# colmap/pycolmap

Measured on AMD Instinct MI355X. Metric: descriptor-pair distances/sec (exhaustive SIFT match: dot + top-2 + ratio + cross-check), higher is better.
Workload: dtype u8 descriptors, int8 MFMA / int32 accumulate; 1 GPU; 500 images x 4096 descriptors, exhaustive match + ratio test + cross-check (BASELINE.json configs[1] at N=1); pairs_total=124750, pairs_per_rank=124750, kernel=auto, matches_rank0=1865611

## Files before the change

### pycolmap_amd/csrc/match_mfma.hip

```cpp
#include <cstdlib>

#include "amc_internal.h"
#include "scan_accept.h"

namespace amc {

typedef int i32x4 __attribute__((ext_vector_type(4)));
typedef __attribute__((address_space(1))) const void gvoid_t;
typedef __attribute__((address_space(3))) void lvoid_t;

constexpr int kBN = 256;
constexpr int kYS = kBN / 32;
constexpr int kUR = 128;
constexpr int kSPB = kUR / 32;
constexpr int kUPC = kBN / kUR;
constexpr int kChunkBytes = kBN * kDim;
constexpr int kW = kSegsPerItem;
constexpr int kXT = kSegRows / 16;
constexpr int kKeyShift = 7, kKeyCarried = 127;

constexpr int kNB = 3;
constexpr int kOffRs = 0;
constexpr int kOffQ = kOffRs + kNB * kBN * 4;
constexpr int kOffB = kOffQ + 16;
constexpr int kLdsBytes = kOffB + kNB * kChunkBytes;
static_assert(kBN == kRowPad, "a chunk is the row padding unit");
static_assert(kUR == 128 && kSPB == 4, "a lane quarter's rows of a block are one 32-row tile; the loop body is one block");
static_assert(kRowPad % kSegRows == 0 && kSegRows % 32 == 0, "segments tile the padded rows");
static_assert(kLdsBytes <= 160 * 1024, "LDS of one CU");
static_assert(sizeof(SegDesc) == 64, "a descriptor is 16 dwords: one per lane of a quarter wave");

enum : int { kDXprep = 0, kDXrs = 2, kDOut = 4, kDList = 6, kDYprep = 8, kDYrs = 10, kDCnt = 12, kDAccword = 13,
             kDYrows = 14 };

__device__ __forceinline__ void mfma_first(i32x4& d, const i32x4& a, const i32x4& b, const i32x4& c) {
    asm volatile("v_mfma_i32_16x16x64_i8 %0, %1, %2, %3" : "=&v"(d) : "v"(a), "v"(b), "v"(c));
}
__device__ __forceinline__ void mfma_acc(i32x4& d, const i32x4& a, const i32x4& b) {
    asm volatile("v_mfma_i32_16x16x64_i8 %0, %1, %2, %0" : "+v"(d) : "v"(a), "v"(b));
}

struct YFrag {
    i32x4 f[2][2];
    i32x4 ci[2];
};

#ifdef AMC_SCAN_STAMPS
constexpr int kStampMaxWG = 1024;
__device__ uint32_t g_scan_stamps[2 * kStampMaxWG * kSegsPerItem * 8];
#define AMC_STAMP() ((uint32_t)__builtin_amdgcn_s_memtime())
#endif

__device__ __noinline__ __attribute__((used)) void copy_part(const uint4* __restrict__ src, uint4* __restrict__ dst,
                                                             unsigned long long b, unsigned long long e, int tid,
                                                             int nthreads) {
    __builtin_assume(tid >= 0 && tid < 1024 && nthreads >= 256 && nthreads <= 512);
    unsigned long long i = b + (unsigned long long)tid;
    const unsigned long long st = (unsigned long long)nthreads;
    for (; i + 3 * st < e; i += 4 * st) {
        const uint4 v0 = src[i], v1 = src[i + st], v2 = src[i + 2 * st], v3 = src[i + 3 * st];
        dst[i] = v0; dst[i + st] = v1; dst[i + 2 * st] = v2; dst[i + 3 * st] = v3;
    }
    for (; i < e; i += st) dst[i] = src[i];
}

template <int MODE>
__global__ __launch_bounds__(64 * kW) void match_mfma_kernel(const SegDesc* __restrict__ segs,
                                                             const uint32_t* __restrict__ nitems_p,
                                                             uint32_t* __restrict__ queue_head,
                                                             uint32_t* __restrict__ accmask,
                                                             const ScanAccept* __restrict__ accept,
                                                             CopyJob job, uint32_t* __restrict__ copy_head) {
    static_assert((kChunkBytes / 1024) % kW == 0 && kYS % (kChunkBytes / 1024 / kW) == 0, "a chunk splits into 1 KiB DMA pieces per wave, dealt evenly over its steps");
    __shared__ __attribute__((aligned(16))) char smem[kLdsBytes];

    const int tid = threadIdx.x;
    const int lane = tid & 63;
    const int wid = __builtin_amdgcn_readfirstlane(tid >> 6);
    const int l15 = lane & 15, lq = lane >> 4;
    volatile uint32_t* s_q = reinterpret_cast<volatile uint32_t*>(smem + kOffQ);
    if constexpr (MODE == 0) {
        if (job.parts) {
            __shared__ uint32_t s_part;
            if (tid == 0) s_part = atomicAdd(copy_head, 1u);
            __syncthreads();
            const uint32_t part = s_part;
            if (part < job.parts)
                copy_part(static_cast<const uint4*>(job.src), static_cast<uint4*>(job.dst), job.n16 * part / job.parts,
                          job.n16 * (part + 1) / job.parts, tid, 64 * kW);
        }
    }
    const uint32_t nitems = *nitems_p;
    const ScanAccept sa = *accept;

    auto load_desc = [&](uint32_t q) -> int {
        int v = 0;
        if (q < nitems && lane < 16) v = reinterpret_cast<const int*>(segs + (size_t)q * kSegsPerItem + wid)[lane];
        return v;
    };
    auto dword = [&](int dv, int f) -> int { return __builtin_amdgcn_readlane(dv, f); };
    auto dptr = [&](int dv, int f) -> const char* {
        const uint64_t lo = (uint32_t)__builtin_amdgcn_readlane(dv, f);
        const uint64_t hi = (uint32_t)__builtin_amdgcn_readlane(dv, f + 1);
        return reinterpret_cast<const char*>(lo | (hi << 32));
    };

    constexpr int kPW = kChunkBytes / 1024 / kW;
    auto stage_piece = [&](const char* yprep, int c, int buf, int ps) __attribute__((always_inline)) {
        const int piece = ps * kW + wid;
        __builtin_amdgcn_global_load_lds((gvoid_t*)(yprep + (size_t)c * kChunkBytes + piece * 1024 + lane * 16),
                                         (lvoid_t*)(smem + kOffB + buf * kChunkBytes + piece * 1024), 16, 0, 0);
    };
    auto stage_rs = [&](const char* yrs, int c, int buf) __attribute__((always_inline)) {
        if (wid == 0)
            __builtin_amdgcn_global_load_lds((gvoid_t*)(yrs + (size_t)c * kBN * 4 + lane * 16),
                                             (lvoid_t*)(smem + kOffRs + buf * kBN * 4), 16, 0, 0);
    };
    auto stage = [&](const char* yprep, const char* yrs, int c, int buf) __attribute__((always_inline)) {
#pragma unroll
        for (int ps = 0; ps < kPW; ++ps) stage_piece(yprep, c, buf, ps);
        stage_rs(yrs, c, buf);
    };

    const int yrow_lane = (kUR / 4) * (l15 >> 2) + (l15 & 3);
    const int ysw_lane = arena_swizzle(yrow_lane);
    const int yoff0 = kOffB + yrow_lane * kDim + ((lq ^ ysw_lane) * 16);
    const int yoff1 = kOffB + yrow_lane * kDim + (((4 + lq) ^ ysw_lane) * 16);
    const int coff = kOffRs + (kUR / 4) * lq * 4;
    auto load_y_part = [&](YFrag& y, int buf, int ys, int part) __attribute__((always_inline)) {
        const int ub = (ys / kSPB) * kUR, sp = ys % kSPB;
        if (part < 2) {
            const int so = buf * kBN * 4 + (ub + 8 * sp) * 4;
            y.ci[part] = *reinterpret_cast<const i32x4*>(smem + (coff + so) + 16 * part);
        } else {
            const int tt = (part - 2) >> 1, s = (part - 2) & 1;
            const int so = buf * kChunkBytes + (ub + 8 * sp) * kDim;
            y.f[tt][s] = *reinterpret_cast<const i32x4*>(smem + ((s ? yoff1 : yoff0) + so) + tt * 4 * kDim);
        }
    };
    auto load_y = [&](YFrag& y, int buf, int ys) __attribute__((always_inline)) {
#pragma unroll
        for (int part = 0; part < 6; ++part) load_y_part(y, buf, ys, part);
    };

    i32x4 xf[kXT][2];
    int best[kXT], sec[kXT], btile[kXT], xterm[kXT], part[kXT];
    auto load_x = [&](int dv) __attribute__((always_inline)) {
        const int cnt = dword(dv, kDCnt);
        const char* xprep = dptr(dv, kDXprep);
        const int* xrs = reinterpret_cast<const int*>(dptr(dv, kDXrs));
#pragma unroll
        for (int xt = 0; xt < kXT; ++xt) {
            const int kl = xt * 16 + l15;
            int row;
            if (MODE == 0) {
                row = kl;
            } else {
                const uint32_t* list = reinterpret_cast<const uint32_t*>(dptr(dv, kDList));
                row = cnt > 0 ? (int)list[min(kl, cnt - 1)] : 0;
            }
            const char* rp = xprep + (size_t)row * kDim;
            const int sw = arena_swizzle(row);
#pragma unroll
            for (int s = 0; s < 2; ++s) xf[xt][s] = *reinterpret_cast<const i32x4*>(rp + (((4 * s + lq) ^ sw) * 16));
            xterm[xt] = xrs[row] - (1 << 21);
            best[xt] = ((-xterm[xt]) << kKeyShift) | kKeyCarried;
            sec[xt] = best[xt];
            btile[xt] = -1;
        }
    };

#ifdef AMC_SCAN_STAMPS
    uint32_t st_a = 0, st_first = 0, st_end = 0, st_sum[5] = {0, 0, 0, 0, 0};
    bool st_prev = false, st_prev_active = false;
    uint32_t* const st_slot = g_scan_stamps + ((size_t)(MODE * kStampMaxWG + min((int)blockIdx.x, kStampMaxWG - 1)) * kW + wid) * 8;
#endif
    if (tid == 0) *s_q = atomicAdd(queue_head, 1u);
    __syncthreads();
    uint32_t q = *s_q;
    int dv = load_desc(q);
    if (q < nitems) {
        stage(dptr(dv, kDYprep), dptr(dv, kDYrs), 0, 0);
        if (dword(dv, kDYrows) > kBN) stage(dptr(dv, kDYprep), dptr(dv, kDYrs), 1, 1);
        if (dword(dv, kDCnt) > 0) load_x(dv);
    }
    __syncthreads();

    while (q < nitems) {
        const char* yprep = dptr(dv, kDYprep);
        const char* yrs = dptr(dv, kDYrs);
        const int yrows_item = dword(dv, kDYrows);
        const int nchunks = (yrows_item + kBN - 1) / kBN;
        const int last_steps = (((yrows_item - (nchunks - 1) * kBN) + 31) / 32 + kSPB - 1) & ~(kSPB - 1);
        const bool active = dword(dv, kDCnt) > 0;
        if (tid == 0) *s_q = atomicAdd(queue_head, 1u);

        i32x4 acc[2][2];
        auto insert = [&](int xt, int code) __attribute__((always_inline)) {
            asm volatile(
                "v_lshl_or_b32 %2, %2, 7, %3\n\t"
                "v_med3_i32 %1, %0, %1, %2\n\t"
                "v_max_i32 %0, %0, %2"
                : "+v"(best[xt]), "+v"(sec[xt]), "+v"(part[xt])
                : "s"(code));
        };
        auto flush = [&](int sb) __attribute__((always_inline)) {
#pragma unroll
            for (int xt = 0; xt < kXT; ++xt) {
                const int c = best[xt] & 127;
                btile[xt] = c != kKeyCarried ? sb * 64 + (126 - c) : btile[xt];
                best[xt] |= kKeyCarried;
            }
        };
        auto phase = [&](i32x4 (&an)[2], const YFrag& y, int xtn, const i32x4 (&ac)[2], int xtc, int sp, int gb)
                         __attribute__((always_inline)) {
            mfma_first(an[0], y.f[0][0], xf[xtn][0], y.ci[0]);
            mfma_first(an[1], y.f[1][0], xf[xtn][0], y.ci[1]);
            __builtin_amdgcn_sched_barrier(0);
            if (xtc == 0 ? sp == 0 : sp == kSPB - 1) {
                insert((xtc + kXT - 1) % kXT, 126 - ((xtc == 0 ? gb - 1 : gb) & 63));
                if (xtc == 0 && gb != 0 && (gb & 63) == 0) flush((gb >> 6) - 1);
                __builtin_amdgcn_sched_barrier(0);
            }
            mfma_acc(an[0], y.f[0][1], xf[xtn][1]);
            mfma_acc(an[1], y.f[1][1], xf[xtn][1]);
            __builtin_amdgcn_sched_barrier(0);
            int t0, t1;
            if (sp == 0)
                asm volatile(
                    "v_max3_i32 %0, %3, %4, %5\n\t"
                    "v_max3_i32 %1, %6, %7, %8\n\t"
                    "v_max3_i32 %0, %0, %9, %10\n\t"
                    "v_max_i32 %2, %0, %1"
                    : "=&v"(t0), "=&v"(t1), "=&v"(part[xtc])
                    : "v"(ac[0][0]), "v"(ac[0][1]), "v"(ac[0][2]), "v"(ac[0][3]), "v"(ac[1][0]), "v"(ac[1][1]),
                      "v"(ac[1][2]), "v"(ac[1][3]));
            else
                asm volatile(
                    "v_max3_i32 %0, %3, %4, %5\n\t"
                    "v_max3_i32 %1, %6, %7, %8\n\t"
                    "v_max3_i32 %0, %0, %9, %10\n\t"
                    "v_max3_i32 %2, %0, %1, %2"
                    : "=&v"(t0), "=&v"(t1), "+v"(part[xtc])
                    : "v"(ac[0][0]), "v"(ac[0][1]), "v"(ac[0][2]), "v"(ac[0][3]), "v"(ac[1][0]), "v"(ac[1][1]),
                      "v"(ac[1][2]), "v"(ac[1][3]));
            __builtin_amdgcn_sched_barrier(0);
        };

        YFrag y0, y1;
        asm volatile("s_waitcnt vmcnt(0)" ::: "memory");
        __syncthreads();
        const uint32_t qn = *s_q;
        const int dvn = load_desc(qn);
#ifdef AMC_SCAN_STAMPS
        {
            const uint32_t now = AMC_STAMP();
            if (st_prev) {
                st_sum[0] += st_a;
                st_sum[1] += now - st_end;
                st_sum[2] += now - st_first;
                st_sum[3] += 1;
                st_sum[4] += st_prev_active ? 1 : 0;
                if (lane == 0) {
#pragma unroll
                    for (int k = 0; k < 5; ++k) st_slot[k] = st_sum[k];
                }
            }
            st_a = 0;
            st_first = now;
        }
#endif
        if (active) {
            load_y(y0, 0, 0);
            mfma_first(acc[0][0], y0.f[0][0], xf[0][0], y0.ci[0]);
            mfma_first(acc[0][1], y0.f[1][0], xf[0][0], y0.ci[1]);
            mfma_acc(acc[0][0], y0.f[0][1], xf[0][1]);
            mfma_acc(acc[0][1], y0.f[1][1], xf[0][1]);
            part[kXT - 1] = -(1 << 24);
            __builtin_amdgcn_sched_barrier(0);
        }
        auto step = [&](YFrag& yc, YFrag& yn, int c, int cb, int nb, int ys, int sp) __attribute__((always_inline)) {
            const bool lastt = sp == kSPB - 1 && ys == kYS - 1;
            const bool cross = lastt && (c + 1 < nchunks);
            const bool fetch = c + 2 < nchunks;
            if (fetch) {
                const int fb = cb == 0 ? 2 : cb - 1;
                constexpr int kEvery = kYS / kPW;
                static_assert(kEvery == 2, "a DMA piece behind every other step");
                if (sp % kEvery == 0) stage_piece(yprep, c + 2, fb, ys / kEvery);
                if (ys == 0) stage_rs(yrs, c + 2, fb);
            }
            if (cross) {
#ifdef AMC_SCAN_STAMPS
                const uint32_t st_t = AMC_STAMP();
#endif
                if (!fetch) asm volatile("s_waitcnt vmcnt(0)" ::: "memory");
                else if (wid == 0) asm volatile("s_waitcnt vmcnt(%0)" ::"n"(kPW + 1) : "memory");
                else asm volatile("s_waitcnt vmcnt(%0)" ::"n"(kPW) : "memory");
                asm volatile("s_barrier" ::: "memory");
#ifdef AMC_SCAN_STAMPS
                st_a += AMC_STAMP() - st_t;
#endif
            }
            if (active) {
                const int nbuf = cross ? nb : cb;
                const int nys = lastt ? (cross ? 0 : ys) : ys + 1;
                const int gb = c * kUPC + ys / kSPB;
#pragma unroll
                for (int xt = 0; xt < kXT; ++xt) {
                    if (xt + 1 < kXT)
                        phase(acc[(xt + 1) & 1], yc, xt + 1, acc[xt & 1], xt, sp, gb);
                    else
                        phase(acc[0], yn, 0, acc[xt & 1], xt, sp, gb);
                    if (xt < 6) {
                        load_y_part(yn, nbuf, nys, xt);
                        __builtin_amdgcn_sched_barrier(0);
                    }
                }
            }
        };
        for (int c = 0, cb = 0; c < nchunks; ++c) {
            const int nb = cb == 2 ? 0 : cb + 1;
            const int yend = (c == nchunks - 1) ? last_steps : kYS;
#pragma unroll 1
            for (int ys = 0; ys < yend; ys += kSPB) {
                step(y0, y1, c, cb, nb, ys, 0);
                step(y1, y0, c, cb, nb, ys + 1, 1);
                step(y0, y1, c, cb, nb, ys + 2, 2);
                step(y1, y0, c, cb, nb, ys + 3, 3);
            }
            cb = nb;
        }
        if (active) {
            const int lastb = (nchunks - 1) * kUPC + last_steps / kSPB - 1;
            insert(kXT - 1, 126 - (lastb & 63));
            flush(lastb >> 6);
#pragma unroll
            for (int xt = 0; xt < kXT; ++xt) {
                best[xt] >>= kKeyShift;
                sec[xt] >>= kKeyShift;
            }
        }
        __syncthreads();
#ifdef AMC_SCAN_STAMPS
        st_end = AMC_STAMP();
        st_prev = true;
        st_prev_active = active;
#endif

        int eb[kXT], es[kXT], et[kXT], ex[kXT];
#pragma unroll
        for (int xt = 0; xt < kXT; ++xt) {
            asm volatile("v_mov_b32 %0, %1" : "=v"(eb[xt]) : "v"(best[xt]));
            asm volatile("v_mov_b32 %0, %1" : "=v"(es[xt]) : "v"(sec[xt]));
            asm volatile("v_mov_b32 %0, %1" : "=v"(et[xt]) : "v"(btile[xt]));
            ex[xt] = xterm[xt];
        }
        if (qn < nitems) {
            stage(dptr(dvn, kDYprep), dptr(dvn, kDYrs), 0, 0);
            if (dword(dvn, kDYrows) > kBN) stage(dptr(dvn, kDYprep), dptr(dvn, kDYrs), 1, 1);
            if (dword(dvn, kDCnt) > 0) load_x(dvn);
        }
        if (active) {
            const int cnt = dword(dv, kDCnt);
            uint32_t bits_lo = 0;
#pragma unroll
            for (int xt = 0; xt < kXT; ++xt) {
                const int kl = xt * 16 + l15;
                int b = eb[xt], s = es[xt], t = et[xt] < 0 ? -1 : et[xt] * kSPB + lq;
#pragma unroll
                for (int m = 16; m <= 32; m <<= 1) {
                    const int ob = __shfl_xor(b, m);
                    const int os = __shfl_xor(s, m);
                    const int ot = __shfl_xor(t, m);
                    const bool ow = (ob > b) || (ob == b && (unsigned)ot < (unsigned)t);
                    s = max(max(s, os), ow ? b : ob);
                    t = ow ? ot : t;
                    b = ow ? ob : b;
                }
                bool acc_bit = false;
                const bool live = lq == 0 && kl < cnt;
                Top2 o;
                o.best_v = (uint32_t)(b + ex[xt]);
                o.best_idx = o.best_v ? (uint32_t)t : 0xFFFFFFFFu;
                o.second_v = (uint32_t)(s + ex[xt]);
                o.pad = 0;
                if (MODE == 0) acc_bit = live && scan_may_accept(sa, o.best_v, o.second_v);
                const uint32_t bits = MODE == 0 ? (uint32_t)__ballot(acc_bit) : 0u;
                if (live && (MODE == 1 || bits != 0)) {
                    Top2* out = reinterpret_cast<Top2*>(const_cast<char*>(dptr(dv, kDOut)));
                    int row = kl;
                    if (MODE == 1) row = (int)reinterpret_cast<const uint32_t*>(dptr(dv, kDList))[kl];
                    out[row] = o;
                }
                if (MODE == 0) {
                    if (xt & 1) {
                        const uint32_t word = bits_lo | (bits << 16);
                        if (lane == 0 && word != 0) accmask[(uint32_t)dword(dv, kDAccword) + (xt >> 1)] = word;
                    } else {
                        bits_lo = bits;
                    }
                }
            }
        }
#ifdef AMC_SCAN_STAMPS
        if (qn >= nitems && lane == 0) {
            st_slot[5] = st_a;
            st_slot[6] = AMC_STAMP() - st_first;
            st_slot[7] = 1;
        }
#endif
        q = qn;
        dv = dvn;
    }
}

__device__ __forceinline__ uint32_t pair_segments(int mode, const ImageDev* imgs, const PairDev& p, uint32_t pi,
                                                  const uint32_t* cand_cnt, uint32_t* nrows_out) {
    const uint32_t nx = mode == 0 ? imgs[p.slot1].rows : cand_cnt[pi];
    const uint32_t ny = imgs[mode == 0 ? p.slot2 : p.slot1].rows;
    *nrows_out = nx;
    return ny ? (nx + kSegRows - 1) / kSegRows : 0u;
}

__global__ __launch_bounds__(256) void seg_count_kernel(int mode, const ImageDev* __restrict__ imgs,
                                                        const PairDev* __restrict__ pairs,
                                                        const uint32_t* __restrict__ order,
                                                        const uint32_t* __restrict__ grp_start,
                                                        const uint32_t* __restrict__ cand_cnt,
                                                        uint32_t* __restrict__ seg_base, uint32_t* __restrict__ grp_segs) {
    __shared__ uint32_t wsum[4];
    const uint32_t g = blockIdx.x, tid = threadIdx.x, lane = tid & 63, wid = tid >> 6;
    const uint32_t i0 = grp_start[g], i1 = grp_start[g + 1];
    uint32_t running = 0;
    for (uint32_t base = i0; base < i1; base += 256) {
        const uint32_t i = base + tid;
        uint32_t s = 0, nr;
        if (i < i1) {
            const uint32_t pi = order[i];
            s = pair_segments(mode, imgs, pairs[pi], pi, cand_cnt, &nr);
        }
        uint32_t inc = s;
#pragma unroll
// ... 54 lines not shown
                                                       const uint32_t* __restrict__ seg_base,
                                                       const uint32_t* __restrict__ grp_segs,
                                                       const uint32_t* __restrict__ grp_item_base,
                                                       Top2* __restrict__ outbuf, SegDesc* __restrict__ segs) {
    const uint32_t g = blockIdx.x, tid = threadIdx.x, lane = tid & 63, wid = blockIdx.y * 4 + (tid >> 6);
    const uint32_t i0 = grp_start[g], i1 = grp_start[g + 1];
    if (i0 >= i1) return;
    const uint32_t total = grp_segs[g];
    if (total == 0) return;
    SegDesc* gs = segs + (size_t)grp_item_base[g] * kSegsPerItem;
    const PairDev p0 = pairs[order[i0]];
    const ImageDev Y = imgs[mode == 0 ? p0.slot2 : p0.slot1];
    for (uint32_t i = i0 + wid; i < i1; i += 4 * kFillY) {
        const uint32_t pi = order[i];
        const PairDev p = pairs[pi];
        uint32_t nx;
        const uint32_t ns = pair_segments(mode, imgs, p, pi, cand_cnt, &nx);
        const ImageDev X = imgs[mode == 0 ? p.slot1 : p.slot2];
        const uint32_t sb = seg_base[i];
        for (uint32_t k = lane; k < ns; k += 64) {
            const uint32_t row0 = k * kSegRows;
            SegDesc d;
            d.yprep = Y.prep;
            d.yrs = Y.rs128;
            d.yrows = Y.rows;
            d.cnt = min(nx - row0, (uint32_t)kSegRows);
            d.pad_ = 0;
            if (mode == 0) {
                d.xprep = X.prep + (size_t)row0 * kDim;
                d.xrs = X.rs128 + row0;
                d.out = outbuf + p.row_off + row0;
                d.list = nullptr;
                d.accword = (uint32_t)((p.row_off + row0) >> 5);
            } else {
                d.xprep = X.prep;
                d.xrs = X.rs128;
                d.out = outbuf + p.col_off;
                d.list = candbuf + p.col_off + row0;
                d.accword = 0;
            }
            gs[sb + k] = d;
        }
    }
    const uint32_t padded = (total + kSegsPerItem - 1) / kSegsPerItem * kSegsPerItem;
    if (blockIdx.y == 0 && tid < padded - total) {
        SegDesc d;
        d.xprep = Y.prep;
        d.xrs = Y.rs128;
        d.out = nullptr;
        d.list = nullptr;
        d.yprep = Y.prep;
        d.yrs = Y.rs128;
        d.cnt = 0;
        d.accword = 0;
        d.yrows = Y.rows;
        d.pad_ = 0;
        gs[total + tid] = d;
    }
}

hipError_t launch_build_segments(int mode, const ImageDev* imgs, const PairDev* pairs, const uint32_t* order,
                                 const uint32_t* grp_start, uint32_t ngroups, const uint32_t* cand_cnt,
                                 const uint32_t* candbuf, Top2* outbuf, uint32_t* seg_base, uint32_t* grp_segs,
                                 uint32_t* grp_item_base, SegDesc* segs, uint32_t* nitems_dev, hipStream_t s) {
    if (ngroups == 0) return memset_async(nitems_dev, 0, sizeof(uint32_t), s);
    hipLaunchKernelGGL(seg_count_kernel, dim3(ngroups), dim3(256), 0, s, mode, imgs, pairs, order, grp_start,
                       cand_cnt, seg_base, grp_segs);
    hipLaunchKernelGGL(seg_scan_kernel, dim3(1), dim3(1024), 0, s, grp_segs, ngroups, grp_item_base, nitems_dev);
    hipLaunchKernelGGL(seg_fill_kernel, dim3(ngroups, kFillY), dim3(256), 0, s, mode, imgs, pairs, order, grp_start,
                       cand_cnt, candbuf, seg_base, grp_segs, grp_item_base, outbuf, segs);
    return hipGetLastError();
}

hipError_t launch_match_mfma(int mode, const SegDesc* segs, const uint32_t* nitems_dev, uint32_t max_items,
                             uint32_t* queue_head, uint32_t* accmask, const ScanAccept* accept_dev, hipStream_t s,
                             const CopyJob& job_in, uint32_t* copy_head) {
    if (max_items == 0) return hipSuccess;
    CopyJob job = (mode == 0 && copy_head) ? job_in : CopyJob();
    hipError_t e = job.parts ? memset_async(copy_head, 0, sizeof(uint32_t), s) : hipSuccess;
    if (e != hipSuccess) return e;
    int dev = 0, cus = 256;
    if ((e = hipGetDevice(&dev)) != hipSuccess) return e;
    if ((e = hipDeviceGetAttribute(&cus, hipDeviceAttributeMultiprocessorCount, dev)) != hipSuccess) return e;
    static const int grid_cap = [] {
        const char* e = std::getenv("AMC_SCAN_GRID");
        return e ? std::atoi(e) : 0;
    }();
    if (grid_cap > 0 && grid_cap < cus) cus = grid_cap;
    const uint32_t grid = max_items < (uint32_t)cus ? max_items : (uint32_t)cus;
    if (job.parts > grid) job.parts = grid;
    if ((e = memset_async(queue_head, 0, sizeof(uint32_t), s)) != hipSuccess) return e;
    if (mode == 0)
        hipLaunchKernelGGL((match_mfma_kernel<0>), dim3(grid), dim3(64 * kW), 0, s, segs, nitems_dev, queue_head,
                           accmask, accept_dev, job, copy_head);
    else
        hipLaunchKernelGGL((match_mfma_kernel<1>), dim3(grid), dim3(64 * kW), 0, s, segs, nitems_dev, queue_head,
                           accmask, accept_dev, job, copy_head);
    return hipGetLastError();
}

}
```

### pycolmap_amd/csrc/amc_internal.h

```cpp
#pragma once

#include <hip/hip_runtime.h>
#include <stdint.h>

#include <algorithm>
#include <cstdlib>
#include <type_traits>
#include <vector>

#include "../../include/amc.h"
#include "guided_region.h"

namespace amc {

constexpr int kDim = AMC_DESC_DIM;
constexpr int kRowPad = 256;
constexpr int kAcosLutSize = 262145;

__host__ __device__ __forceinline__ constexpr uint32_t arena_swizzle(uint32_t row) {
    return ((row >> 1) & 1u) | (((row >> 5) & 3u) << 1);
}

struct ImageDev {
    const uint8_t* raw;
// ... 196 lines not shown

    hipError_t start() { return made_ != hipSuccess ? made_ : hipEventRecord(ab_[0], s_); }
    hipError_t stop(double& ms) {
        hipError_t e = hipEventRecord(ab_[1], s_);
        if (e == hipSuccess) e = hipEventSynchronize(ab_[1]);
        return e == hipSuccess ? add_elapsed(ab_[0], ab_[1], ms) : e;
    }
    hipError_t span_begin() {
        hipEvent_t two[2];
        if (const hipError_t e = create_events(two, 2)) return e;
        spans_.insert(spans_.end(), two, two + 2);
        return hipEventRecord(two[0], s_);
    }
    hipError_t span_end() { return hipEventRecord(spans_.back(), s_); }
    hipError_t spans(double& ms) const {
        for (size_t i = 0; i + 1 < spans_.size(); i += 2)
            if (const hipError_t e = add_elapsed(spans_[i], spans_[i + 1], ms)) return e;
        return hipSuccess;
    }

  private:
    static hipError_t add_elapsed(hipEvent_t a, hipEvent_t b, double& ms) {
        float f = 0.f;
        const hipError_t e = hipEventElapsedTime(&f, a, b);
        if (e == hipSuccess) ms += f;
        return e;
    }
    hipStream_t s_;
    hipEvent_t ab_[2] = {nullptr, nullptr};
    hipError_t made_;
    std::vector<hipEvent_t> spans_;
};

struct Batches {
    std::vector<size_t> start{0};
    uint64_t most_items = 0, most_elems = 0;
    size_t count() const { return start.size() - 1; }
};
inline Batches split_batches(const uint64_t* offsets, size_t n, uint64_t max_items, uint64_t max_elems,
                             uint64_t factor = 1) {
    Batches b;
    for (size_t i = 0; i < n;) {
        size_t j = i + 1;
        while (j < n && j - i < max_items && (offsets[j + 1] - offsets[i]) * factor <= max_elems) ++j;
        b.most_items = std::max<uint64_t>(b.most_items, j - i);
        b.most_elems = std::max<uint64_t>(b.most_elems, offsets[j] - offsets[i]);
        b.start.push_back(j);
        i = j;
    }
    return b;
}

struct CtxView {
    int device;
    hipStream_t stream;
    const uint32_t* resident;
    uint64_t resident_rows;
};
CtxView ctx_view(amc_ctx* c);
struct TvgPair;
struct VerifyResident {
    size_t npairs = 0;
    uint64_t total = 0;
    const amc_tvg* tvg = nullptr;
    const uint8_t* mask = nullptr;
    const uint64_t* moff = nullptr;
    const TvgPair* tp = nullptr;
    const uint32_t* matches = nullptr;
};
VerifyResident verify_resident(amc_ctx* c);

hipError_t memset_async(void* p, int value, size_t bytes, hipStream_t s);
hipError_t memcpy_async(void* dst, const void* src, size_t bytes, hipMemcpyKind kind, hipStream_t s);

hipError_t launch_prep(const uint8_t* raw, uint8_t* prep, int32_t* rs128, uint32_t rows_pad,
                 uint32_t* maxsq_out, hipStream_t s);

hipError_t launch_match_dot4(const ImageDev* imgs, const PairDev* pairs, const Dot4Work* work,
                       uint32_t nwork, Top2* rowbuf, Top2* colbuf, const GuidedDev* guided, hipStream_t s);
hipError_t launch_match_guided_grid(const ImageDev* imgs, const GridDev* grids, const PairDev* pairs, const Dot4Work* work,
                              uint32_t nwork, Top2* rowbuf, Top2* colbuf, const GuidedDev* guided, hipStream_t s);

constexpr int kSegRows = 128;
constexpr int kSegsPerItem = 8;
struct alignas(64) SegDesc {
    const uint8_t* xprep;
    const int32_t* xrs;
    Top2* out;
    const uint32_t* list;
    const uint8_t* yprep;
    const int32_t* yrs;
    uint32_t cnt;
    uint32_t accword;
    uint32_t yrows;
    uint32_t pad_;
};
__device__ __forceinline__ bool one_way_accepts(const Top2 t, const float* __restrict__ lut,
                                                float max_ratio, float max_distance) {
    if (t.best_v == 0u) return false;
    const float a_best = lut[min(t.best_v, 262144u)];
    if (a_best > max_distance) return false;
    const float a_second = lut[min(t.second_v, 262144u)];
    if (a_best >= max_ratio * a_second) return false;
    return true;
}

hipError_t launch_build_segments(int mode, const ImageDev* imgs, const PairDev* pairs, const uint32_t* order,
                           const uint32_t* grp_start, uint32_t ngroups, const uint32_t* cand_cnt,
                           const uint32_t* candbuf, Top2* outbuf, uint32_t* seg_base, uint32_t* grp_segs,
                           uint32_t* grp_item_base, SegDesc* segs, uint32_t* nitems_dev, hipStream_t s);
struct ScanAccept;
struct CopyJob {
    const void* src = nullptr;
    void* dst = nullptr;
    unsigned long long n16 = 0;
    uint32_t parts = 0, pad_ = 0;
};
hipError_t launch_match_mfma(int mode, const SegDesc* segs, const uint32_t* nitems_dev, uint32_t max_items,
                       uint32_t* queue_head, uint32_t* accmask, const ScanAccept* accept_dev, hipStream_t s,
                       const CopyJob& job = CopyJob(), uint32_t* copy_head = nullptr);

hipError_t launch_resolve_index(int side, const ImageDev* imgs, const PairDev* pairs, uint32_t npairs,
                          Top2* table, uint32_t* accmask, const float* acos_lut, FinalizeParams fp,
                          const uint32_t* cand_cnt, const uint32_t* candbuf, uint32_t* err_count,
                          bool grouped, const uint32_t* order, uint32_t norder, hipStream_t s);
uint32_t resolve_grouped_max_rows();
constexpr uint32_t kSelectMaxCols = 1u << 20;

hipError_t launch_select_candidates(const ImageDev* imgs, const PairDev* pairs, uint32_t npairs, uint32_t max_cols,
                              const Top2* rowbuf, const uint32_t* accmask, const float* acos_lut,
                              FinalizeParams fp, uint32_t* cand_cnt, uint32_t* candbuf, hipStream_t s);

hipError_t launch_finalize(const ImageDev* imgs, const PairDev* pairs, uint32_t npairs,
                     const Top2* rowbuf, const Top2* colbuf, uint32_t* accmask,
                     const float* acos_lut, FinalizeParams fp, uint32_t* cursor, uint32_t capacity,
                     uint32_t* pair_off, uint32_t* pair_cnt, uint32_t* matches, hipStream_t s);

hipError_t launch_host_copy(void* dst_pinned, const void* src_dev, size_t bytes, hipStream_t s);
hipError_t launch_reorder_matches(const uint32_t* src_off, const uint32_t* cnt, const uint64_t* dst_off, uint32_t npairs,
                            const uint32_t* src, uint32_t* dst, hipStream_t s);

struct CameraDev {
    int32_t model_id;
    int32_t has_prior;
    uint64_t width, height;
    double params[12];
};
struct TvgImage {
    const float* kp;
    const double* kp64;
    const double* kpn;
    uint32_t rows;
    uint32_t pad;
    CameraDev cam;
};
hipError_t launch_undistort(const float* kp, const double* kp64, uint32_t rows, const CameraDev& cam, double* kpn,
                            hipStream_t s);
hipError_t launch_project(const double* uv, uint32_t n, const CameraDev& cam, double* xy, hipStream_t s);
struct TvgPair {
    uint32_t slot1, slot2;
    uint64_t match_off;
    uint64_t mask_off;
    uint32_t M;
    uint32_t tab_off[3];
    uint32_t orig;
};
struct PosePair {
// ... 83 lines not shown
```

### pycolmap_amd/csrc/amc_match.hip

```cpp
#include <algorithm>
#include <chrono>
#include <cstdio>
#include <cstdlib>
#include <cstring>
#include <limits>
#include <memory>
#include <new>
#include <vector>

#include "amc_ctx.h"

using namespace amc;

namespace {

struct ResultPriv {
    std::vector<uint64_t> offsets;
    PinBuf<uint32_t> matches;
    std::shared_ptr<PinnedPool> pool;
    ~ResultPriv() {
        if (pool) pool->give_back(std::move(matches));
    }
};

// ... 65 lines not shown
                return api_fail(AMC_E_STATE, "amc_match_guided_pairs: pair %zu: float32 keypoints (one per descriptor) "
                                "must be uploaded for both images", i);
            guided_grid_setup(g, a.grid, b.grid, guided_dense_only);
        }
    }
    HIPCHK(hipSetDevice(c->device));
    hipStream_t st = c->stream;

    if (c->table_dirty) {
        HIPCHK(c->d_imgs.ensure(c->slots.size()));
        std::vector<ImageDev> t(c->slots.size());
        for (size_t i = 0; i < t.size(); ++i) t[i] = c->slots[i].dev;
        if (!t.empty())
            HIPCHK(hipMemcpy(c->d_imgs.p, t.data(), t.size() * sizeof(ImageDev),
                             hipMemcpyHostToDevice));
        HIPCHK(c->d_grids.ensure(c->slots.size()));
        std::vector<GridDev> gt(c->slots.size());
        for (size_t i = 0; i < gt.size(); ++i) gt[i] = c->slots[i].grid;
        if (!gt.empty())
            HIPCHK(hipMemcpy(c->d_grids.p, gt.data(), gt.size() * sizeof(GridDev), hipMemcpyHostToDevice));
        c->table_dirty = false;
    }

    const float max_ratio_f = (float)o.max_ratio;
    FinalizeParams fp;
    fp.max_ratio = max_ratio_f;
    fp.max_distance = (float)o.max_distance;
    fp.cross_check = o.cross_check ? 1 : 0;
    fp.reserved = 0;

    if (!c->accept_valid || std::memcmp(&c->accept_ratio, &fp.max_ratio, sizeof(float)) != 0 ||
        std::memcmp(&c->accept_distance, &fp.max_distance, sizeof(float)) != 0) {
        c->h_accept = build_scan_accept(c->h_lut.data(), (uint32_t)c->h_lut.size(), fp.max_ratio, fp.max_distance);
        if (accept_trivial) c->h_accept.trivial = 1;
        if (!c->d_accept) HIPCHK(hipMalloc(reinterpret_cast<void**>(&c->d_accept), sizeof(ScanAccept)));
        HIPCHK(hipStreamSynchronize(st));
        HIPCHK(hipMemcpy(c->d_accept, &c->h_accept, sizeof(ScanAccept), hipMemcpyHostToDevice));
        c->accept_ratio = fp.max_ratio;
        c->accept_distance = fp.max_distance;
        c->accept_valid = true;
    }
    HIPCHK(hipEventRecord(c->ev[0], st));
    ResultPriv* priv = new (std::nothrow) ResultPriv();
    if (!priv) return api_fail(AMC_E_NOMEM, "amc_match_pairs: out of host memory");
    priv->offsets.assign(npairs + 1, 0);
    priv->pool = c->result_pool;
    priv->matches = c->result_pool->acquire();
    size_t keep_used = 0;
    c->resident_matches = 0;
    c->vres = amc::VerifyResident{};
    if (keep_off) keep_off->assign(npairs, 0);

    const size_t mfma_max_cols = kSelectMaxCols;

    uint64_t num_dist = 0, n_mfma = 0, n_dot4 = 0, n_grid = 0;
    double kernel_ms = 0.0, cross_ms = 0.0;
    uint32_t kernel_launches = 0;

    int rc = AMC_OK;
    auto hc = [&](hipError_t e, const char* what) {
        if (e != hipSuccess && rc == AMC_OK)
            rc = api_fail(AMC_E_HIP, "amc_match_pairs: %s: %s", what, hipGetErrorString(e));
        return e == hipSuccess;
    };
    const size_t max_entries = batch_entries ? batch_entries : kMaxTop2Entries;

    struct Batch {
        size_t begin = 0, end = 0, nb = 0, top_rows = 0, top_cols = 0, cap = 0;
        size_t row_off = 0, nwork = 0, nord = 0, nwork_grid = 0;
        uint32_t max_cols = 0;
        size_t ngrp = 0, ngrp2 = 0, seg_cap = 0;
        int set = 0;
        uint32_t total = 0;
        bool grouped_resolve = true;
    };
    uint64_t rows_carved = 0, rows_collected = 0;
    const int d2h_mode = !d2h_env ? 0 : (std::strcmp(d2h_env, "memcpy") == 0 ? 2 : (std::strcmp(d2h_env, "stream") == 0 ? 1 : 0));
    struct PendingCopy {
        void* dst = nullptr;
        const void* src = nullptr;
        size_t bytes = 0;
        int set = -1;
    } pending;
    constexpr uint32_t kCopyParts = 8;
    auto sync_batch_streams = [&](const char* what) { return hc(hipStreamSynchronize(st), what); };
    const bool hook_split = batch_hook && hook_split_mode != 0;
    const size_t hook_split_min_pairs = hook_split_mode == 2 ? 2 : 4096;
    auto carve = [&](size_t begin, int set) {
        Batch b;
        b.begin = b.end = begin;
        b.set = set;
        size_t limit = max_entries;
        const uint64_t rows_left = rows_total - rows_carved;
        if (begin > 0 && rows_left <= max_entries && rows_left > max_entries / 4)
            limit = (size_t)(rows_left - max_entries / 4);
        if (begin == 0 && hook_split && rows_total <= max_entries && npairs >= hook_split_min_pairs)
            limit = (size_t)(rows_total * 6 / 10);
        while (b.end < npairs) {
            const Slot& x = c->slots[slot1[b.end]];
            const Slot& y = c->slots[slot2[b.end]];
            const size_t nr = x.dev.rows_pad, nc = y.dev.rows_pad;
            const size_t mc = o.cross_check ? std::min(x.dev.rows, y.dev.rows) : x.dev.rows;
            if (b.end > b.begin && (b.top_rows + nr > limit || b.top_cols + nc > max_entries ||
                                    b.cap + mc > kMaxMatchCap || b.end - b.begin >= (1u << 24)))
                break;
            b.top_rows += nr; b.top_cols += nc; b.cap += mc; ++b.end;
        }
        b.nb = b.end - b.begin;
        rows_carved += b.top_rows;
        return b;
    };
    auto prepare = [&](Batch& b) {
        const int k = b.set;
        const size_t nb = b.nb, begin = b.begin;
        if (!hc(c->h_pairs[k].ensure(nb), "pinned pairs") || !hc(c->h_order[k].ensure(nb), "pinned order") ||
            !hc(c->h_order2[k].ensure(nb), "pinned order2") || !hc(c->h_pair_off[k].ensure(nb), "pinned pair_off") ||
            !hc(c->h_pair_cnt[k].ensure(nb), "pinned pair_cnt") || !hc(c->h_bscalars[k].ensure(16), "pinned scalars"))
            return false;
        std::vector<uint8_t> want_mfma(nb, 0);
        for (size_t i = 0; i < nb; ++i) {
            const Slot& x = c->slots[slot1[begin + i]];
            const Slot& y = c->slots[slot2[begin + i]];
            const bool nonempty = x.dev.rows > 0 && y.dev.rows > 0;
            want_mfma[i] = nonempty && o.kernel != AMC_KERNEL_DOT4 && !geoms &&
                           (!o.cross_check || y.dev.rows_pad <= mfma_max_cols);
        }
        PairDev* hp = c->h_pairs[k].p;
        size_t row_off = 0, col_off = 0, nwork = 0, nord = 0;
        b.grouped_resolve = !resolve_ungrouped;
        for (size_t i = 0; i < nb; ++i) {
            const Slot& x = c->slots[slot1[begin + i]];
            const Slot& y = c->slots[slot2[begin + i]];
            const bool nonempty = x.dev.rows > 0 && y.dev.rows > 0;
            if (o.kernel == AMC_KERNEL_MFMA && nonempty && !want_mfma[i]) {
                rc = api_fail(AMC_E_INVALID,
                              "amc_match_pairs: kernel=MFMA forced but pair %zu is not eligible "
                              "(rows_pad=%u, cols_pad=%u > %zu)", begin + i, x.dev.rows_pad,
                              y.dev.rows_pad, mfma_max_cols);
                return false;
            }
            PairDev& pd = hp[i];
            pd.slot1 = slot1[begin + i];
            pd.slot2 = slot2[begin + i];
            pd.mode = want_mfma[i] ? 1u : 0u;
            pd.pad = 0;
            pd.row_off = row_off;
            pd.col_off = col_off;
            row_off += x.dev.rows_pad;
            col_off += y.dev.rows_pad;
            num_dist += (uint64_t)x.dev.rows * y.dev.rows;
            if (!nonempty) continue;
            if (want_mfma[i]) {
                c->h_order[k].p[nord++] = (uint32_t)i;
                ++n_mfma;
                b.max_cols = std::max(b.max_cols, y.dev.rows);
                if (std::max(x.dev.rows_pad, y.dev.rows_pad) > resolve_grouped_max_rows()) b.grouped_resolve = false;
            } else {
                nwork += (x.dev.rows + 63) / 64;
                if (o.cross_check) nwork += (y.dev.rows + 63) / 64;
                if (geoms && h_guided[begin + i].grid_ok) ++n_grid; else ++n_dot4;
            }
        }
        if (nord) {
            const size_t nslots = c->slots.size();
            std::vector<uint32_t> cnt(nslots + 1), tmp(nord);
            auto by_slot = [&](const uint32_t* src, uint32_t* dst, bool key_is_slot2) {
                std::fill(cnt.begin(), cnt.end(), 0u);
// ... 410 lines not shown
```

Measured before the change: 13250 billion distances/s.

## Traverse Y chunks serpentine across consecutive items to reuse staged LDS buffers

```diff
diff --git a/profiles/serpentine/recipes/loop_counts.py b/profiles/serpentine/recipes/loop_counts.py
--- /dev/null
+++ b/profiles/serpentine/recipes/loop_counts.py
@@ -0,0 +1,27 @@
+import sys,re,collections
+def kernels(path):
+    txt=open(path).read().split('\n')
+    out={};cur=None
+    for l in txt:
+        m=re.match(r'^(_ZN3amc17match_mfma_kernelILi(\d)E\S*):',l)
+        if m: cur=m.group(2); out[cur]=[]
+        elif l.startswith('.Lfunc_end'): cur=None
+        elif cur is not None: out[cur].append(l)
+    return out
+def blocks(lines):
+    b=[];cur=['entry',[]]
+    for l in lines:
+        m=re.match(r'^(\.LBB\S+):',l)
+        if m: b.append(cur);cur=[m.group(1),[]]
+        else:
+            t=l.strip()
+            if t and not t.startswith(';') and not t.startswith('.'): cur[1].append(t)
+    b.append(cur);return b
+for path in sys.argv[1:]:
+    for mode,lines in kernels(path).items():
+        for name,ins in blocks(lines):
+            n=sum(i.startswith('v_mfma') for i in ins)
+            if n>=32:
+                c=collections.Counter(i.split()[0] for i in ins)
+                key=['v_mfma_i32_16x16x64_i8','v_max3_i32','v_max_i32','v_med3_i32','v_lshl_or_b32','ds_read_b128','s_nop','s_waitcnt','s_barrier','global_load_lds_dwordx4','v_mov_b32','v_readlane_b32','v_writelane_b32']
+                print(path.split('/')[-1],'MODE',mode,name,len(ins),{k:c[k] for k in key}, 'salu',sum(v for k,v in c.items() if k.startswith('s_') and k not in('s_nop','s_waitcnt','s_barrier')), 'valu_other',{k:v for k,v in c.items() if k.startswith('v_') and k not in key})
diff --git a/pycolmap_amd/csrc/match_mfma.hip b/pycolmap_amd/csrc/match_mfma.hip
--- a/pycolmap_amd/csrc/match_mfma.hip
+++ b/pycolmap_amd/csrc/match_mfma.hip
@@ -46,8 +46,8 @@
 };
 
 #ifdef AMC_SCAN_STAMPS
-constexpr int kStampMaxWG = 1024;
-__device__ uint32_t g_scan_stamps[2 * kStampMaxWG * kSegsPerItem * 8];
+constexpr int kStampMaxWG = 1024, kStampDw = 10;
+__device__ uint32_t g_scan_stamps[2 * kStampMaxWG * kSegsPerItem * kStampDw];
 #define AMC_STAMP() ((uint32_t)__builtin_amdgcn_s_memtime())
 #endif
 
@@ -171,13 +171,15 @@
     };
 
 #ifdef AMC_SCAN_STAMPS
-    uint32_t st_a = 0, st_first = 0, st_end = 0, st_sum[5] = {0, 0, 0, 0, 0};
+    uint32_t st_a = 0, st_first = 0, st_end = 0, st_chunks = 0, st_sum[7] = {0, 0, 0, 0, 0, 0, 0};
     bool st_prev = false, st_prev_active = false;
-    uint32_t* const st_slot = g_scan_stamps + ((size_t)(MODE * kStampMaxWG + min((int)blockIdx.x, kStampMaxWG - 1)) * kW + wid) * 8;
+    uint32_t* const st_slot = g_scan_stamps + ((size_t)(MODE * kStampMaxWG + min((int)blockIdx.x, kStampMaxWG - 1)) * kW + wid) * kStampDw;
 #endif
+    int cb = 0, dstep = 1;
+    bool fresh = true;
     if (tid == 0) *s_q = atomicAdd(queue_head, 1u);
     __syncthreads();
-    uint32_t q = *s_q;
+    uint32_t q = __builtin_amdgcn_readfirstlane(*s_q);
     int dv = load_desc(q);
     if (q < nitems) {
         stage(dptr(dv, kDYprep), dptr(dv, kDYrs), 0, 0);
@@ -212,13 +214,13 @@
                 best[xt] |= kKeyCarried;
             }
         };
-        auto phase = [&](i32x4 (&an)[2], const YFrag& y, int xtn, const i32x4 (&ac)[2], int xtc, int sp, int gb)
-                         __attribute__((always_inline)) {
+        auto phase = [&](i32x4 (&an)[2], const YFrag& y, int xtn, const i32x4 (&ac)[2], int xtc, int sp, int gb,
+                         int pcode) __attribute__((always_inline)) {
             mfma_first(an[0], y.f[0][0], xf[xtn][0], y.ci[0]);
             mfma_first(an[1], y.f[1][0], xf[xtn][0], y.ci[1]);
             __builtin_amdgcn_sched_barrier(0);
             if (xtc == 0 ? sp == 0 : sp == kSPB - 1) {
-                insert((xtc + kXT - 1) % kXT, 126 - ((xtc == 0 ? gb - 1 : gb) & 63));
+                insert((xtc + kXT - 1) % kXT, xtc == 0 ? pcode : 126 - (gb & 63));
                 if (xtc == 0 && gb != 0 && (gb & 63) == 0) flush((gb >> 6) - 1);
                 __builtin_amdgcn_sched_barrier(0);
             }
@@ -250,7 +252,7 @@
         YFrag y0, y1;
         asm volatile("s_waitcnt vmcnt(0)" ::: "memory");
         __syncthreads();
-        const uint32_t qn = *s_q;
+        const uint32_t qn = __builtin_amdgcn_readfirstlane(*s_q);
         const int dvn = load_desc(qn);
 #ifdef AMC_SCAN_STAMPS
         {
@@ -261,17 +263,22 @@
                 st_sum[2] += now - st_first;
                 st_sum[3] += 1;
                 st_sum[4] += st_prev_active ? 1 : 0;
+                st_sum[5] += fresh ? 0 : 1;
+                st_sum[6] += st_chunks;
                 if (lane == 0) {
 #pragma unroll
                     for (int k = 0; k < 5; ++k) st_slot[k] = st_sum[k];
+                    st_slot[8] = st_sum[5];
+                    st_slot[9] = st_sum[6];
                 }
             }
+            st_chunks = fresh ? nchunks : (nchunks > kNB ? nchunks - kNB : 0);
             st_a = 0;
             st_first = now;
         }
 #endif
         if (active) {
-            load_y(y0, 0, 0);
+            load_y(y0, cb, 0);
             mfma_first(acc[0][0], y0.f[0][0], xf[0][0], y0.ci[0]);
             mfma_first(acc[0][1], y0.f[1][0], xf[0][0], y0.ci[1]);
             mfma_acc(acc[0][0], y0.f[0][1], xf[0][1]);
@@ -279,16 +286,16 @@
             part[kXT - 1] = -(1 << 24);
             __builtin_amdgcn_sched_barrier(0);
         }
-        auto step = [&](YFrag& yc, YFrag& yn, int c, int cb, int nb, int ys, int sp) __attribute__((always_inline)) {
-            const bool lastt = sp == kSPB - 1 && ys == kYS - 1;
-            const bool cross = lastt && (c + 1 < nchunks);
-            const bool fetch = c + 2 < nchunks;
+        auto step = [&](YFrag& yc, YFrag& yn, int c, int cb, int nb, int ys, int sp, int yend, bool more, bool fetch,
+                        int pcode) __attribute__((always_inline)) {
+            const bool lastt = sp == kSPB - 1 && ys == yend - 1;
+            const bool cross = lastt && more;
             if (fetch) {
-                const int fb = cb == 0 ? 2 : cb - 1;
+                const int fb = 3 - cb - nb;
                 constexpr int kEvery = kYS / kPW;
                 static_assert(kEvery == 2, "a DMA piece behind every other step");
-                if (sp % kEvery == 0) stage_piece(yprep, c + 2, fb, ys / kEvery);
-                if (ys == 0) stage_rs(yrs, c + 2, fb);
+                if (sp % kEvery == 0) stage_piece(yprep, c + 2 * dstep, fb, ys / kEvery);
+                if (ys == 0) stage_rs(yrs, c + 2 * dstep, fb);
             }
             if (cross) {
 #ifdef AMC_SCAN_STAMPS
@@ -309,9 +316,9 @@
 #pragma unroll
                 for (int xt = 0; xt < kXT; ++xt) {
                     if (xt + 1 < kXT)
-                        phase(acc[(xt + 1) & 1], yc, xt + 1, acc[xt & 1], xt, sp, gb);
+                        phase(acc[(xt + 1) & 1], yc, xt + 1, acc[xt & 1], xt, sp, gb, pcode);
                     else
-                        phase(acc[0], yn, 0, acc[xt & 1], xt, sp, gb);
+                        phase(acc[0], yn, 0, acc[xt & 1], xt, sp, gb, pcode);
                     if (xt < 6) {
                         load_y_part(yn, nbuf, nys, xt);
                         __builtin_amdgcn_sched_barrier(0);
@@ -319,21 +326,28 @@
                 }
             }
         };
-        for (int c = 0, cb = 0; c < nchunks; ++c) {
-            const int nb = cb == 2 ? 0 : cb + 1;
+        int pcode = 0;
+        for (int k = 0, c = dstep > 0 ? 0 : nchunks - 1; k < nchunks; ++k) {
+            const int nb = dstep > 0 ? (cb == 2 ? 0 : cb + 1) : (cb == 0 ? 2 : cb - 1);
             const int yend = (c == nchunks - 1) ? last_steps : kYS;
+            const bool more = k + 1 < nchunks;
+            const bool fetch = k + 2 < nchunks && (fresh || k > 0);
 #pragma unroll 1
             for (int ys = 0; ys < yend; ys += kSPB) {
-                step(y0, y1, c, cb, nb, ys, 0);
-                step(y1, y0, c, cb, nb, ys + 1, 1);
-                step(y0, y1, c, cb, nb, ys + 2, 2);
-                step(y1, y0, c, cb, nb, ys + 3, 3);
-            }
-            cb = nb;
+                step(y0, y1, c, cb, nb, ys, 0, yend, more, fetch, pcode);
+                step(y1, y0, c, cb, nb, ys + 1, 1, yend, more, fetch, pcode);
+                step(y0, y1, c, cb, nb, ys + 2, 2, yend, more, fetch, pcode);
+                step(y1, y0, c, cb, nb, ys + 3, 3, yend, more, fetch, pcode);
+                pcode = 126 - ((c * kUPC + ys / kSPB) & 63);
+            }
+            if (more) {
+                cb = nb;
+                c += dstep;
+            }
         }
         if (active) {
             const int lastb = (nchunks - 1) * kUPC + last_steps / kSPB - 1;
-            insert(kXT - 1, 126 - (lastb & 63));
+            insert(kXT - 1, pcode);
             flush(lastb >> 6);
 #pragma unroll
             for (int xt = 0; xt < kXT; ++xt) {
@@ -357,8 +371,17 @@
             ex[xt] = xterm[xt];
         }
         if (qn < nitems) {
-            stage(dptr(dvn, kDYprep), dptr(dvn, kDYrs), 0, 0);
-            if (dword(dvn, kDYrows) > kBN) stage(dptr(dvn, kDYprep), dptr(dvn, kDYrs), 1, 1);
+            const int yrows_n = dword(dvn, kDYrows);
+            if (dptr(dvn, kDYprep) == dptr(dv, kDYprep) && yrows_n == dword(dv, kDYrows) && yrows_n <= 64 * kUR) {
+                dstep = -dstep;
+                fresh = false;
+            } else {
+                cb = 0;
+                dstep = 1;
+                fresh = true;
+                stage(dptr(dvn, kDYprep), dptr(dvn, kDYrs), 0, 0);
+                if (yrows_n > kBN) stage(dptr(dvn, kDYprep), dptr(dvn, kDYrs), 1, 1);
+            }
             if (dword(dvn, kDCnt) > 0) load_x(dvn);
         }
         if (active) {
```

Result: no change. 13360 billion distances/s, median of 6 (+0.8%).

## Run two 4-wave workgroups per CU with 128-row chunks and deeper DMA ring

Applied to the files above, without the earlier changes.

```diff
diff --git a/pycolmap_amd/csrc/amc_internal.h b/pycolmap_amd/csrc/amc_internal.h
--- a/pycolmap_amd/csrc/amc_internal.h
+++ b/pycolmap_amd/csrc/amc_internal.h
@@ -302,7 +302,7 @@
                               uint32_t nwork, Top2* rowbuf, Top2* colbuf, const GuidedDev* guided, hipStream_t s);
 
 constexpr int kSegRows = 128;
-constexpr int kSegsPerItem = 8;
+constexpr int kSegsPerItem = 4;
 struct alignas(64) SegDesc {
     const uint8_t* xprep;
     const int32_t* xrs;
diff --git a/pycolmap_amd/csrc/amc_match.hip b/pycolmap_amd/csrc/amc_match.hip
--- a/pycolmap_amd/csrc/amc_match.hip
+++ b/pycolmap_amd/csrc/amc_match.hip
@@ -171,7 +171,7 @@
         size_t bytes = 0;
         int set = -1;
     } pending;
-    constexpr uint32_t kCopyParts = 8;
+    constexpr uint32_t kCopyParts = 64 / kSegsPerItem;
     auto sync_batch_streams = [&](const char* what) { return hc(hipStreamSynchronize(st), what); };
     const bool hook_split = batch_hook && hook_split_mode != 0;
     const size_t hook_split_min_pairs = hook_split_mode == 2 ? 2 : 4096;
diff --git a/pycolmap_amd/csrc/match_mfma.hip b/pycolmap_amd/csrc/match_mfma.hip
--- a/pycolmap_amd/csrc/match_mfma.hip
+++ b/pycolmap_amd/csrc/match_mfma.hip
@@ -9,25 +9,27 @@
 typedef __attribute__((address_space(1))) const void gvoid_t;
 typedef __attribute__((address_space(3))) void lvoid_t;
 
-constexpr int kBN = 256;
+constexpr int kBN = 128;
 constexpr int kYS = kBN / 32;
 constexpr int kUR = 128;
 constexpr int kSPB = kUR / 32;
-constexpr int kUPC = kBN / kUR;
 constexpr int kChunkBytes = kBN * kDim;
 constexpr int kW = kSegsPerItem;
+constexpr int kWGPerCU = 2;
 constexpr int kXT = kSegRows / 16;
 constexpr int kKeyShift = 7, kKeyCarried = 127;
 
-constexpr int kNB = 3;
+constexpr int kNB = 4;
 constexpr int kOffRs = 0;
 constexpr int kOffQ = kOffRs + kNB * kBN * 4;
 constexpr int kOffB = kOffQ + 16;
 constexpr int kLdsBytes = kOffB + kNB * kChunkBytes;
-static_assert(kBN == kRowPad, "a chunk is the row padding unit");
-static_assert(kUR == 128 && kSPB == 4, "a lane quarter's rows of a block are one 32-row tile; the loop body is one block");
+static_assert(kRowPad % kBN == 0, "a chunk divides the row padding: every chunk that holds a row lies inside the padded image");
+static_assert(kUR == 128 && kSPB == 4 && kBN == kUR, "a lane quarter's rows of a block are one 32-row tile; the loop body is one block, which is one chunk");
 static_assert(kRowPad % kSegRows == 0 && kSegRows % 32 == 0, "segments tile the padded rows");
-static_assert(kLdsBytes <= 160 * 1024, "LDS of one CU");
+static_assert((kNB & (kNB - 1)) == 0, "the ring position is taken modulo kNB with a mask");
+static_assert(kWGPerCU * (kLdsBytes + 16) <= 160 * 1024, "LDS of one CU holds two workgroups (and their copy-part slots)");
+static_assert(kW == 4, "one wave of a workgroup per SIMD");
 static_assert(sizeof(SegDesc) == 64, "a descriptor is 16 dwords: one per lane of a quarter wave");
 
 enum : int { kDXprep = 0, kDXrs = 2, kDOut = 4, kDList = 6, kDYprep = 8, kDYrs = 10, kDCnt = 12, kDAccword = 13,
@@ -65,13 +67,12 @@
 }
 
 template <int MODE>
-__global__ __launch_bounds__(64 * kW) void match_mfma_kernel(const SegDesc* __restrict__ segs,
-                                                             const uint32_t* __restrict__ nitems_p,
-                                                             uint32_t* __restrict__ queue_head,
-                                                             uint32_t* __restrict__ accmask,
-                                                             const ScanAccept* __restrict__ accept,
-                                                             CopyJob job, uint32_t* __restrict__ copy_head) {
-    static_assert((kChunkBytes / 1024) % kW == 0 && kYS % (kChunkBytes / 1024 / kW) == 0, "a chunk splits into 1 KiB DMA pieces per wave, dealt evenly over its steps");
+__global__ __launch_bounds__(64 * kW) __attribute__((amdgpu_waves_per_eu(kWGPerCU, kWGPerCU)))
+void match_mfma_kernel(const SegDesc* __restrict__ segs, const uint32_t* __restrict__ nitems_p,
+                       uint32_t* __restrict__ queue_head, uint32_t* __restrict__ accmask,
+                       const ScanAccept* __restrict__ accept, CopyJob job, uint32_t* __restrict__ copy_head) {
+    static_assert(kChunkBytes / 1024 == kW * kYS, "a chunk splits into 1 KiB DMA pieces, one per wave and step");
+    static_assert(kBN * 4 == 512, "a chunk's rs128 block is half a wave's DMA");
     __shared__ __attribute__((aligned(16))) char smem[kLdsBytes];
 
     const int tid = threadIdx.x;
@@ -112,7 +113,7 @@
                                          (lvoid_t*)(smem + kOffB + buf * kChunkBytes + piece * 1024), 16, 0, 0);
     };
     auto stage_rs = [&](const char* yrs, int c, int buf) __attribute__((always_inline)) {
-        if (wid == 0)
+        if (wid == 0 && lane < kBN / 4)
             __builtin_amdgcn_global_load_lds((gvoid_t*)(yrs + (size_t)c * kBN * 4 + lane * 16),
                                              (lvoid_t*)(smem + kOffRs + buf * kBN * 4), 16, 0, 0);
     };
@@ -120,6 +121,15 @@
 #pragma unroll
         for (int ps = 0; ps < kPW; ++ps) stage_piece(yprep, c, buf, ps);
         stage_rs(yrs, c, buf);
+    };
+    auto stage_head = [&](int dv) __attribute__((always_inline)) {
+        const char* yprep = dptr(dv, kDYprep);
+        const char* yrs = dptr(dv, kDYrs);
+        const int yrows = dword(dv, kDYrows);
+        stage(yprep, yrs, 0, 0);
+#pragma unroll
+        for (int c = 1; c < kNB - 1; ++c)
+            if (yrows > c * kBN) stage(yprep, yrs, c, c);
     };
 
     const int yrow_lane = (kUR / 4) * (l15 >> 2) + (l15 & 3);
@@ -180,8 +190,7 @@
     uint32_t q = *s_q;
     int dv = load_desc(q);
     if (q < nitems) {
-        stage(dptr(dv, kDYprep), dptr(dv, kDYrs), 0, 0);
-        if (dword(dv, kDYrows) > kBN) stage(dptr(dv, kDYprep), dptr(dv, kDYrs), 1, 1);
+        stage_head(dv);
         if (dword(dv, kDCnt) > 0) load_x(dv);
     }
     __syncthreads();
@@ -189,9 +198,7 @@
     while (q < nitems) {
         const char* yprep = dptr(dv, kDYprep);
         const char* yrs = dptr(dv, kDYrs);
-        const int yrows_item = dword(dv, kDYrows);
-        const int nchunks = (yrows_item + kBN - 1) / kBN;
-        const int last_steps = (((yrows_item - (nchunks - 1) * kBN) + 31) / 32 + kSPB - 1) & ~(kSPB - 1);
+        const int nchunks = (dword(dv, kDYrows) + kBN - 1) / kBN;
         const bool active = dword(dv, kDCnt) > 0;
         if (tid == 0) *s_q = atomicAdd(queue_head, 1u);
 
@@ -279,24 +286,31 @@
             part[kXT - 1] = -(1 << 24);
             __builtin_amdgcn_sched_barrier(0);
         }
-        auto step = [&](YFrag& yc, YFrag& yn, int c, int cb, int nb, int ys, int sp) __attribute__((always_inline)) {
-            const bool lastt = sp == kSPB - 1 && ys == kYS - 1;
+        auto step = [&](YFrag& yc, YFrag& yn, int c, int cb, int nb, int ys) __attribute__((always_inline)) {
+            const int sp = ys;
+            const bool lastt = ys == kYS - 1;
             const bool cross = lastt && (c + 1 < nchunks);
-            const bool fetch = c + 2 < nchunks;
+            const bool fetch = c + kNB - 1 < nchunks;
+            static_assert(kPW == kYS, "one DMA piece per wave and step");
             if (fetch) {
-                const int fb = cb == 0 ? 2 : cb - 1;
-                constexpr int kEvery = kYS / kPW;
-                static_assert(kEvery == 2, "a DMA piece behind every other step");
-                if (sp % kEvery == 0) stage_piece(yprep, c + 2, fb, ys / kEvery);
-                if (ys == 0) stage_rs(yrs, c + 2, fb);
+                const int fb = (cb + kNB - 1) & (kNB - 1);
+                stage_piece(yprep, c + kNB - 1, fb, ys);
+                if (ys == 0) stage_rs(yrs, c + kNB - 1, fb);
             }
             if (cross) {
 #ifdef AMC_SCAN_STAMPS
                 const uint32_t st_t = AMC_STAMP();
 #endif
-                if (!fetch) asm volatile("s_waitcnt vmcnt(0)" ::: "memory");
-                else if (wid == 0) asm volatile("s_waitcnt vmcnt(%0)" ::"n"(kPW + 1) : "memory");
-                else asm volatile("s_waitcnt vmcnt(%0)" ::"n"(kPW) : "memory");
+                static_assert(kNB == 4, "the counted waits below are written out for three chunks ahead");
+                if (fetch) {
+                    if (wid == 0) asm volatile("s_waitcnt vmcnt(%0)" ::"n"(2 * kPW + 2) : "memory");
+                    else asm volatile("s_waitcnt vmcnt(%0)" ::"n"(2 * kPW) : "memory");
+                } else if (c + 2 < nchunks) {
+                    if (wid == 0) asm volatile("s_waitcnt vmcnt(%0)" ::"n"(kPW + 1) : "memory");
+                    else asm volatile("s_waitcnt vmcnt(%0)" ::"n"(kPW) : "memory");
+                } else {
+                    asm volatile("s_waitcnt vmcnt(0)" ::: "memory");
+                }
                 asm volatile("s_barrier" ::: "memory");
 #ifdef AMC_SCAN_STAMPS
                 st_a += AMC_STAMP() - st_t;
@@ -305,7 +319,7 @@
             if (active) {
                 const int nbuf = cross ? nb : cb;
                 const int nys = lastt ? (cross ? 0 : ys) : ys + 1;
-                const int gb = c * kUPC + ys / kSPB;
+                const int gb = c;
 #pragma unroll
                 for (int xt = 0; xt < kXT; ++xt) {
                     if (xt + 1 < kXT)
@@ -319,20 +333,16 @@
                 }
             }
         };
-        for (int c = 0, cb = 0; c < nchunks; ++c) {
-            const int nb = cb == 2 ? 0 : cb + 1;
-            const int yend = (c == nchunks - 1) ? last_steps : kYS;
 #pragma unroll 1
-            for (int ys = 0; ys < yend; ys += kSPB) {
-                step(y0, y1, c, cb, nb, ys, 0);
-                step(y1, y0, c, cb, nb, ys + 1, 1);
-                step(y0, y1, c, cb, nb, ys + 2, 2);
-                step(y1, y0, c, cb, nb, ys + 3, 3);
-            }
-            cb = nb;
+        for (int c = 0; c < nchunks; ++c) {
+            const int cb = c & (kNB - 1), nb = (c + 1) & (kNB - 1);
+            step(y0, y1, c, cb, nb, 0);
+            step(y1, y0, c, cb, nb, 1);
+            step(y0, y1, c, cb, nb, 2);
+            step(y1, y0, c, cb, nb, 3);
         }
         if (active) {
-            const int lastb = (nchunks - 1) * kUPC + last_steps / kSPB - 1;
+            const int lastb = nchunks - 1;
             insert(kXT - 1, 126 - (lastb & 63));
             flush(lastb >> 6);
 #pragma unroll
@@ -357,8 +367,7 @@
             ex[xt] = xterm[xt];
         }
         if (qn < nitems) {
-            stage(dptr(dvn, kDYprep), dptr(dvn, kDYrs), 0, 0);
-            if (dword(dvn, kDYrows) > kBN) stage(dptr(dvn, kDYprep), dptr(dvn, kDYrs), 1, 1);
+            stage_head(dvn);
             if (dword(dvn, kDCnt) > 0) load_x(dvn);
         }
         if (active) {
@@ -579,12 +588,21 @@
     int dev = 0, cus = 256;
     if ((e = hipGetDevice(&dev)) != hipSuccess) return e;
     if ((e = hipDeviceGetAttribute(&cus, hipDeviceAttributeMultiprocessorCount, dev)) != hipSuccess) return e;
+    static const hipError_t occupancy = [] {
+        int n0 = 0, n1 = 0;
+        hipError_t oe = hipOccupancyMaxActiveBlocksPerMultiprocessor(&n0, match_mfma_kernel<0>, 64 * kW, 0);
+        if (oe == hipSuccess) oe = hipOccupancyMaxActiveBlocksPerMultiprocessor(&n1, match_mfma_kernel<1>, 64 * kW, 0);
+        if (oe != hipSuccess) return oe;
+        return n0 >= kWGPerCU && n1 >= kWGPerCU ? hipSuccess : hipErrorLaunchOutOfResources;
+    }();
+    if (occupancy != hipSuccess) return occupancy;
+    int wgs = kWGPerCU * cus;
     static const int grid_cap = [] {
         const char* e = std::getenv("AMC_SCAN_GRID");
         return e ? std::atoi(e) : 0;
     }();
-    if (grid_cap > 0 && grid_cap < cus) cus = grid_cap;
-    const uint32_t grid = max_items < (uint32_t)cus ? max_items : (uint32_t)cus;
+    if (grid_cap > 0 && grid_cap < wgs) wgs = grid_cap;
+    const uint32_t grid = max_items < (uint32_t)wgs ? max_items : (uint32_t)wgs;
     if (job.parts > grid) job.parts = grid;
     if ((e = memset_async(queue_head, 0, sizeof(uint32_t), s)) != hipSuccess) return e;
     if (mode == 0)
```

Result: faster. 13160 billion distances/s before, 13590 billion distances/s after, median of 6 (+3.3%).
